# unclearness/vacancy

Measured on AMD Instinct MI355X. Metric: Mvoxel*views/s (Carve), higher is better.
Workload: dtype f32

## Files before the change

### vacancy_amd/csrc/carve_fused.h

```cpp
#pragma once
#include <algorithm>
#include <cstdint>

#include "carve_common.h"

namespace vcy {

#ifndef VCY_WG_WAVES
#define VCY_WG_WAVES 4
#endif
constexpr int kWgWaves = VCY_WG_WAVES;
constexpr int BX = 8 * kWgWaves, BY = 8, BZ = 8;
constexpr int WX = 8;
constexpr int kMaxFusedViews = 64;
constexpr int kTileRaw = 16;
constexpr int kRawBuffers = 2;
template <int TQ>
constexpr int tile_f4_per_wave() { return TQ == kTileRaw ? kRawBuffers * 64 : TQ; }
constexpr int kTileBig = 512;
constexpr int kBigPixels = 4 * kTileBig;

constexpr int kCoopSdfPitch = 8 * VCY_WG_WAVES + 4;
template <typename CountT>
constexpr int coop_cnt_pitch() { return 8 * VCY_WG_WAVES + 16 / (int)sizeof(CountT); }
// ... 56 lines not shown
  float ub;
  int sure;
};
static_assert(sizeof(TileInfo) == 56, "row_lds_bytes_per_wave");

constexpr int kUpdateWaUnitWeight = 2;

struct FootprintRecord {
  uint32_t w0, w1;
};

__device__ __forceinline__ FootprintRecord pack_footprint(const TileInfo& ti, const ViewParams& v) {
  uint32_t b = __float_as_uint(ti.ub);
  if (!(fabsf(ti.ub) <= 3.402823466e+38f)) b = 0x7f800000u;
  else if (b & 0x80000000u) b &= ~63u;
  else b = (b + 63u) & ~63u;
  FootprintRecord r;
  const int tx1 = ti.tx0 + ti.tw - 1, ty1 = ti.ty0 + ti.th - 1;
  r.w0 = b | (uint32_t)ti.th | (ti.nq && tx1 == v.roi_max_xi ? 16u : 0u) | (ti.nq && ty1 == v.roi_max_yi ? 32u : 0u);
  r.w1 = ti.nq ? ((uint32_t)ti.tx0 | ((uint32_t)ti.ty0 << 13) | ((uint32_t)ti.tw << 26) | ((uint32_t)ti.sure << 30)) : 0u;
  return r;
}

__device__ __forceinline__ TileInfo unpack_footprint(const FootprintRecord r) {
  TileInfo ti;
  const int tw = (int)((r.w1 >> 26) & 15u), th = (int)(r.w0 & 15u);
  const int tx0 = (int)(r.w1 & 8191u), ty0 = (int)((r.w1 >> 13) & 8191u);
  ti.ub = __uint_as_float(r.w0 & ~63u);
  ti.sure = (int)(r.w1 >> 30);
  ti.tx0 = tx0, ti.ty0 = ty0, ti.tw = tw, ti.th = (tw ? th : 0), ti.nq = tw * th;
  ti.pitchf = tw ? 16.0f : 0.0f;
  ti.inv_tw = tw ? 0.0625f : 1.0f;
  ti.base = tw ? -(ty0 * 16 + tx0) : 0;
  if (tw) {
    const int tx1 = tx0 + tw - 1, ty1 = ty0 + th - 1;
    ti.lo_x = (float)tx0, ti.lo_y = (float)ty0;
    ti.hi_x = (r.w0 & 16u) ? (float)tx1 : __uint_as_float(__float_as_uint((float)(tx1 + 1)) - 1u);
    ti.hi_y = (r.w0 & 32u) ? (float)ty1 : __uint_as_float(__float_as_uint((float)(ty1 + 1)) - 1u);
  } else {
    ti.lo_x = ti.lo_y = INFINITY;
    ti.hi_x = ti.hi_y = -INFINITY;
    ti.ub = INFINITY;
    ti.sure = 0;
  }
  return ti;
}

struct FastDivU32 {
  uint32_t d, m, s1, s2;
};
__device__ __forceinline__ uint32_t fast_div_u32(uint32_t n, const FastDivU32& f) {
  const uint32_t t = __umulhi(n, f.m);
  return (t + ((n - t) >> f.s1)) >> f.s2;
}
inline FastDivU32 make_fast_div_u32(uint32_t d) {
  FastDivU32 f;
  uint32_t l = 0;
  while ((1ull << l) < d) ++l;
  f.d = d;
  f.m = (uint32_t)((((1ull << l) - d) << 32) / d + 1);
  f.s1 = l < 1 ? l : 1;
  f.s2 = l < 1 ? 0 : l - 1;
  return f;
}

struct BlockDecode {
  int total;
  int layer, q, rem, dealt;
// ... 63 lines not shown
```

### vacancy_amd/csrc/carve_fused_device.h

```cpp
#pragma once
#include "carve_fused.h"

namespace vcy {
namespace {

#define VCY_SETPRIO(n) __builtin_amdgcn_s_setprio(n)

#ifdef VCY_PHASE_TIMING
__device__ unsigned long long g_phase_ticks[256][16];
#define VCY_PT_DECL unsigned long long pt_last = __builtin_amdgcn_s_memtime(), pt_acc[16] = {0, 0, 0, 0, 0, 0, 0, 0, 0, 0, 0, 0, 0, 0, 0, 0}
#define VCY_PT(slot)                                                  \
  do {                                                                \
    const unsigned long long t_ = __builtin_amdgcn_s_memtime();       \
    pt_acc[slot] += t_ - pt_last;                                     \
    pt_last = t_;                                                     \
  } while (0)
#define VCY_PT_COUNT(slot) pt_acc[slot] += 1
#define VCY_PT_FLUSH(lane_)                                                                         \
  do {                                                                                              \
    if ((lane_) == 0)                                                                               \
      for (int q_ = 0; q_ < 16; ++q_) atomicAdd(&g_phase_ticks[blockIdx.x & 255][q_], pt_acc[q_]);  \
  } while (0)
#else
#define VCY_PT_DECL
// ... 120 lines not shown
typedef float f4 __attribute__((ext_vector_type(4)));
typedef f4 __attribute__((address_space(3))) lds_float4;

template <int UPDATE>
__device__ __forceinline__ bool apply_sample(bool ok, float dist, float wgt, float& s, float& fn) {
  const float f1 = fn + 1.0f;
  float avg;
  if (UPDATE == kUpdateWaUnitWeight) {
    avg = (fn * s + dist) * rcp_count(f1);
  } else {
    avg = (wgt * fn * s + wgt * dist) * div_fast(1.0f, wgt * f1);
  }
  const float ns = (fn < 1.0f) ? dist : avg;
  s = ok ? ns : s;
  fn = ok ? f1 : fn;
  return ok;
}

__device__ __forceinline__ int div_small(int q, float inv) { return (int)(((float)q + 0.5f) * inv); }

typedef float __attribute__((address_space(3))) lds_float;
typedef uint32_t __attribute__((address_space(3))) lds_u32;

__device__ __forceinline__ void raw_prefetch(const ViewParams& v, const TileInfo& ti, int lane, float* buf) {
#ifdef VCY_FLOOR_NO_TILE_LOADS
  return;
#endif
  asm volatile("" : "+v"(lane));
  const int nq = __builtin_amdgcn_readfirstlane(ti.nq);
  if (nq == 0) return;
  const int th = __builtin_amdgcn_readfirstlane(ti.th);
  const int tx0 = __builtin_amdgcn_readfirstlane(ti.tx0);
  const int ty0 = __builtin_amdgcn_readfirstlane(ti.ty0);
  gfloat_ptr img = (gfloat_ptr)v.sdf;
  const unsigned width = (unsigned)v.width;
  lds_float* dst = (lds_float*)buf;
  if (tx0 + 15 <= v.roi_max_xi && ty0 + 15 <= v.roi_max_yi) {
    const unsigned lane_off = __umul24(width, (unsigned)lane >> 4) + ((unsigned)lane & 15u);
    gfloat_ptr base = img + (__umul24(width, (unsigned)ty0) + (unsigned)tx0);
#pragma unroll
    for (int r = 0; r < 4; ++r) {
      if (4 * r <= th)
        __builtin_amdgcn_global_load_lds(base + (size_t)(4 * r) * width + lane_off, dst + 64 * r, 4, 0, 0);
    }
    return;
  }
  const unsigned xx = (unsigned)min(tx0 + (lane & 15), v.roi_max_xi);
  const int yl = ty0 + (lane >> 4);
#pragma unroll
  for (int r = 0; r < 4; ++r) {
    if (4 * r <= th) {
      const unsigned yy = (unsigned)min(yl + 4 * r, v.roi_max_yi);
      __builtin_amdgcn_global_load_lds(img + (__umul24(width, yy) + xx), dst + 64 * r, 4, 0, 0);
    }
  }
}

__device__ __forceinline__ void raw_tile_wait() { asm volatile("s_waitcnt vmcnt(0)" ::: "memory"); }

__device__ __forceinline__ float wave_min(float v) {
#define VCY_DPP_MIN(CTRL) "s_nop 1\n\tv_min_f32_dpp %0, %0, %0 " CTRL "\n\t"
  asm volatile(VCY_DPP_MIN("quad_perm:[1,0,3,2] row_mask:0xf bank_mask:0xf")
               VCY_DPP_MIN("quad_perm:[2,3,0,1] row_mask:0xf bank_mask:0xf")
               VCY_DPP_MIN("row_half_mirror row_mask:0xf bank_mask:0xf")
               VCY_DPP_MIN("row_mirror row_mask:0xf bank_mask:0xf")
               VCY_DPP_MIN("row_bcast:15 row_mask:0xa bank_mask:0xf")
               VCY_DPP_MIN("row_bcast:31 row_mask:0xc bank_mask:0xf")
               : "+v"(v));
#undef VCY_DPP_MIN
  return __uint_as_float(__builtin_amdgcn_readlane(__float_as_uint(v), 63));
}

__device__ __forceinline__ void tile_fill(const ViewParams& v, const TileInfo& ti, int lane, float* tile) {
  const int nq = __builtin_amdgcn_readfirstlane(ti.nq);
  if (nq == 0) return;
  const int tw = __builtin_amdgcn_readfirstlane(ti.tw), th = __builtin_amdgcn_readfirstlane(ti.th);
  const int tx0 = __builtin_amdgcn_readfirstlane(ti.tx0);
// ... 208 lines not shown
  uint32_t w32[sizeof(TileInfo) / 4];
  __builtin_memcpy(w32, &ti, sizeof(TileInfo));
  lds_u32* dst = tinfo_lds + vi * (int)(sizeof(TileInfo) / 4);
#pragma unroll
  for (int q = 0; q < (int)(sizeof(TileInfo) / 4); ++q) dst[q] = w32[q];
}

template <bool SAMEF, int TQ, bool GEN>
__device__ __attribute__((noinline)) float brick_footprints(const FusedView* __restrict__ views, int nviews, int lane,
                                                            float xl, float xh, float yl, float yh, float zl_, float zh,
                                                            bool is_ortho, bool outside_max, bool want_bound,
                                                            bool want_lower, lds_u32* tinfo_lds) {
  float ub_lane = INFINITY;
  if (lane < nviews) {
    const FusedView fv = load_fused_view(views, lane);
    const TileInfo ti = footprint_of<SAMEF, TQ, GEN>(fv, xl, xh, yl, yh, zl_, zh, is_ortho, outside_max, want_bound,
                                                     want_lower);
    store_tile_info(tinfo_lds, lane, ti);
    ub_lane = ti.ub;
  }
  return ub_lane;
}

}
}
```

### vacancy_amd/csrc/carve_fused_kernel.h

```cpp
#pragma once
#include <cstdio>
#include <cstdlib>
#include <type_traits>

#include "carve_fused_device.h"

namespace vcy {
namespace {

template <int UPDATE, bool CHECKMAX, int TQ, bool GEN, int NB>
constexpr int carve_waves_per_simd() {
  if (NB > 1) return NB > 2 ? 4 : 5;
  if (GEN || CHECKMAX || TQ != kTileRaw || UPDATE == VCY_UPDATE_WEIGHTED_AVERAGE) return VCY_WAVES_CHECKED;
  if (UPDATE == kUpdateWaUnitWeight) return NB == 0 ? VCY_WAVES_WA_ONE : VCY_WAVES_WA;
  return NB == 0 ? VCY_WAVES_ONE : VCY_WAVES;
}
template <typename CountT, int UPDATE, bool TRUNC, bool SAMEF, bool CHECKMAX, int TQ, bool GEN, int DIV, int NB = 1>
__global__ __launch_bounds__(64 * (NB > 1 ? kRowWaves : kWgWaves))
__attribute__((amdgpu_waves_per_eu(NB > 1 ? 1 : carve_waves_per_simd<UPDATE, CHECKMAX, TQ, GEN, NB>(),
                                   carve_waves_per_simd<UPDATE, CHECKMAX, TQ, GEN, NB>()))) void carve_fused_kernel(GridParams g,
                                                          const FusedView* __restrict__ views,
                                                          const float* __restrict__ c0_all,
                                                          int nviews_arg, ModeParams mode, int nbx,
                                                          int nby, BlockDecode bd, int cull_enabled, int state_flags,
                                                          const FootprintRecord* __restrict__ records,
                                                          int64_t nbricks, float* __restrict__ brick_min,
                                                          const int* __restrict__ wg_list,
                                                          unsigned long long* __restrict__ pair_count) {
  constexpr bool kOne = NB == 0;
  constexpr bool kOneRegs = kOne;
  const int nviews = kOne ? 1 : nviews_arg;
  const int fresh = state_flags & kStateFresh;
  const bool implied = (state_flags & kStateCountImplied) != 0;
  const bool coop = NB <= 1 && (kWgWaves == 4 || kWgWaves == 8) && (state_flags & kStateCoopStore) != 0;
  const bool nt_store = (state_flags & kStateStreamStore) != 0;
  constexpr bool kRows = NB > 1;
  static_assert(!kRows || (TQ == kTileRaw && !CHECKMAX), "the few-view flavour: raw tiles, no update limit in reach");
  extern __shared__ float4 fused_lds[];
  constexpr bool kRaw = TQ == kTileRaw;
  constexpr int kTileF4 = NB == 0 ? 64 : tile_f4_per_wave<TQ>();
  constexpr bool kNeedBound = TRUNC || UPDATE == VCY_UPDATE_MAX;

  VCY_SETPRIO(3);
  const int tid = threadIdx.x;
  const int wave = __builtin_amdgcn_readfirstlane(tid >> 6), lane = tid & 63;
  VCY_PT_DECL;
  constexpr size_t kRowWaveBytes = kRows ? row_lds_bytes_per_wave<CountT, NB>() : 0;
  static_assert(kRowWaveBytes % 16 == 0, "wave regions are 16-byte aligned");
  float4* tile = kRows ? (float4*)((char*)fused_lds + wave * kRowWaveBytes) : fused_lds + wave * kTileF4;
  TileInfo* tinfo = kRows ? (TileInfo*)((char*)tile + kRawBuffers * 1024)
                          : (TileInfo*)(fused_lds + kWgWaves * kTileF4) + wave * nviews;
  float* stage_s = (float*)((char*)tinfo + NB * kRowMaxViews * sizeof(TileInfo));
  CountT* stage_n = (CountT*)(stage_s + NB * 64 * WX);
  typedef unsigned long long __attribute__((address_space(3))) lds_u64_row;
  lds_u64_row* stage_mask = (lds_u64_row*)(unsigned long long*)(stage_n + NB * 64 * WX);
  static_assert((sizeof(TileInfo) * kWgWaves) % 16 == 0, "alignment of the cooperative write-back's staging");
  typedef CountT CountVec8 __attribute__((ext_vector_type(WX)));
  typedef CountVec8 __attribute__((address_space(3))) lds_countvec;
  typedef unsigned long long __attribute__((address_space(3))) lds_u64;
  float* coop_s = NB == 0 ? (float*)(fused_lds + kWgWaves * kTileF4)
                          : (float*)((TileInfo*)(fused_lds + kWgWaves * kTileF4) + kWgWaves * nviews);
  CountT* coop_n = (CountT*)(coop_s + 64 * kCoopSdfPitch);
  lds_u64* coop_mask = (lds_u64*)(unsigned long long*)(coop_n + 64 * coop_cnt_pitch<CountT>());
  auto coop_leave = [&]() {
    if (coop) {
      if (lane == 0) coop_mask[wave] = 0ull, coop_mask[kWgWaves + wave] = 0ull;
      __builtin_amdgcn_fence(__ATOMIC_RELEASE, "workgroup");
    }
  };
  TileInfo ti_one;
  auto tile_of = [&](int p) -> const TileInfo& {
    if constexpr (kOneRegs) return ti_one;
    else return tinfo[p];
  };
  int cur = 0;
  auto raw_buf = [&](int b) -> float* { return (float*)tile + 256 * b; };
  const int ly = lane & (BY - 1), lz = lane >> 3;
  int b = kRows ? ((int)(blockIdx.x & 7u) + 8 * (kRowWaves * (int)(blockIdx.x >> 3) + wave)) : (int)blockIdx.x;
  const int* list_entry = nullptr;
  int list_live = 0;
  FootprintRecord list_rec;
  list_rec.w0 = 0u, list_rec.w1 = 0u;
  if (wg_list != nullptr) {
    if (kRows) b = (int)blockIdx.x * kRowWaves + wave;
    if (b >= wg_list[0]) return;
    if (kOne && (state_flags & kStateListRecords) != 0) {
      list_entry = wg_list + 2 + (int64_t)b * kLiveEntryWords;
      typedef uint32_t u32x2 __attribute__((ext_vector_type(2)));
      typedef const u32x2 __attribute__((address_space(1))) * gent_ptr;
      const u32x2 head = ((gent_ptr)list_entry)[0], mine = ((gent_ptr)list_entry)[1 + wave];
      b = __builtin_amdgcn_readfirstlane((int)head.x);
      list_live = __builtin_amdgcn_readfirstlane((int)head.y);
      list_rec.w0 = (uint32_t)__builtin_amdgcn_readfirstlane((int)mine.x);
      list_rec.w1 = (uint32_t)__builtin_amdgcn_readfirstlane((int)mine.y);
    } else {
      b = wg_list[1 + b];
    }
  } else {
    if (kRows && b >= bd.total) return;
// ... 69 lines not shown
      rec.w0 = raw.x, rec.w1 = raw.y;
      const TileInfo ti = unpack_footprint(rec);
      store_tile_info((lds_u32*)tinfo, lane, ti);
      ub_lane = ti.ub;
    }
  } else if constexpr (kOneRegs) {
    typedef uint32_t u32x2 __attribute__((ext_vector_type(2)));
    typedef const u32x2 __attribute__((address_space(1))) * grec_ptr;
    FootprintRecord rec;
    if (list_entry != nullptr) {
      rec = list_rec;
    } else {
      const u32x2 raw = ((grec_ptr)records)[brick_lin];
      rec.w0 = (uint32_t)__builtin_amdgcn_readfirstlane((int)raw.x), rec.w1 = (uint32_t)__builtin_amdgcn_readfirstlane((int)raw.y);
    }
    ti_one = unpack_footprint(rec);
    ub_lane = ti_one.ub;
  } else if (kRaw && records != nullptr) {
    ub_lane = INFINITY;
    if (lane < nviews) {
      typedef uint32_t u32x2 __attribute__((ext_vector_type(2)));
      typedef const u32x2 __attribute__((address_space(1))) * grec_ptr;
      const u32x2 raw = ((grec_ptr)records)[(int64_t)lane * nbricks + brick_lin];
      FootprintRecord rec;
      rec.w0 = raw.x, rec.w1 = raw.y;
      const TileInfo ti = unpack_footprint(rec);
      store_tile_info((lds_u32*)tinfo, lane, ti);
      ub_lane = ti.ub;
    }
  } else {
    const int x_lo = min(x_first, g.nx - 1), x_hi = min(x_first + WX - 1, g.nx - 1);
    const int y_hi = min(by * BY + BY - 1, g.ny - 1);
    const int z_hi = min(zl0 + BZ - 1, g.nz_local - 1);
    ub_lane = brick_footprints<SAMEF, TQ, GEN>(views, nviews, lane, g.px[x_lo], g.px[x_hi], g.py[by * BY], g.py[y_hi],
                                               g.pz[g.z0 + zl0], g.pz[g.z0 + z_hi], mode.ortho != 0,
                                               mode.outside == VCY_OUTSIDE_MAX, want_bound,
                                               want_bound && TRUNC && UPDATE != VCY_UPDATE_MAX, (lds_u32*)tinfo);
  }
  wave_lds_fence();
#if defined(VCY_DEV_EXIT_AT) && VCY_DEV_EXIT_AT == 2
  {
    coop_leave();
    return;
  }
#endif
  const unsigned long long view_mask = kRows ? __ballot(pair_valid) : ((nviews >= 64) ? ~0ull : ((1ull << nviews) - 1ull));
  unsigned long long live = view_mask;
  if (want_bound && !fresh && !(kOne && list_entry != nullptr)) {
    const bool have_min = UPDATE == VCY_UPDATE_MAX && (state_flags & kStateBrickMinValid) != 0 && brick_min != nullptr;
    if (TRUNC || have_min) {
      bool drop0 = TRUNC && ub_lane < -1.0f;
      if (have_min) {
        float smin0;
        if constexpr (kRows) smin0 = pair_valid ? brick_min[brick_seg + pair_j] : 0.0f;
        else smin0 = ((cfloat_ptr)brick_min)[brick_lin];
        drop0 = drop0 || ub_lane <= smin0;
      }
      live = __ballot(!drop0) & view_mask;
      if (live == 0ull) {
        coop_leave();
        return;
      }
    }
  }
#ifdef VCY_PHASE_TIMING
  {
    asm volatile("" ::"v"(ub_lane));
    const unsigned long long t_ = __builtin_amdgcn_s_memtime();
    pt_acc[13] += t_ - pt_last;
  }
#endif

#if defined(VCY_DEV_EXIT_AT) && VCY_DEV_EXIT_AT == 3
  {
    coop_leave();
    return;
  }
#endif
  CountT* __restrict__ cnt = (CountT*)g.cnt;
  constexpr bool kFloatCount = UPDATE != VCY_UPDATE_MAX;
  typedef typename std::conditional<kFloatCount, float, int>::type NT;
  float s[WX];
  NT n[WX];
  const int64_t row0 = ((int64_t)zl * g.ny + y) * g.nx;
  int vi_pre = -1;
  auto prefetch_first_tile = [&]() {
    if constexpr (kRaw) {
      const bool listed_live = kOne && list_entry != nullptr;
      const bool have_min = UPDATE == VCY_UPDATE_MAX && !fresh && (state_flags & kStateBrickMinValid) != 0 && brick_min != nullptr;
      if (!(fresh || UPDATE != VCY_UPDATE_MAX || !want_bound || have_min || listed_live)) return;
      bool drop = false;
      if (want_bound && !listed_live) {
        if (TRUNC) drop = ub_lane < -1.0f;
        if (have_min) {
          const float smin0 = ((cfloat_ptr)brick_min)[brick_lin];
          if (smin0 != kInvalidSdf) drop = drop || ub_lane <= smin0;
        }
      }
      const unsigned long long lp = __ballot(!drop) & view_mask;
      vi_pre = lp ? (__ffsll((long long)lp) - 1) : nviews;
      if (vi_pre < nviews) raw_prefetch(views[vi_pre].v, tile_of(vi_pre), lane, raw_buf(0));
    }
  };
  const bool vec_io = (g.nx & (WX - 1)) == 0;
  typedef CountT CountVec __attribute__((ext_vector_type(WX)));
  if constexpr (kRows) {
#pragma unroll
    for (int k = 0; k < WX; ++k) {
      s[k] = kInvalidSdf;
      n[k] = (NT)0;
    }
    if (lane < NB) stage_mask[lane] = 0ull;
    if (!fresh) {
      const int yl = min(by * BY + (lane >> 3), g.ny - 1);
      const unsigned off_s = (unsigned)yl * (unsigned)g.nx + (unsigned)(lane & 7);
      constexpr int kCntPerDword = 4 / (int)sizeof(CountT);
      constexpr int kCntDwordsPerRow = WX / kCntPerDword;
      constexpr int kCntRowsPerReq = 64 / kCntDwordsPerRow;
      constexpr int kCntReqs = 64 / kCntRowsPerReq;
      const int crow = lane / kCntDwordsPerRow;
      typedef const CountT __attribute__((address_space(1))) * gcnt_ptr;
#pragma unroll
      for (int j = 0; j < NB; ++j) {
        if (((live >> (8 * j)) & 0xffull) == 0ull) continue;
        const int xb = x_seg + j * WX;
#pragma unroll
        for (int r = 0; r < BZ; ++r) {
          const int zr = min(zl0 + r, g.nz_local - 1);
          gfloat_ptr src = (gfloat_ptr)g.sdf + ((int64_t)zr * g.ny * g.nx + xb);
          __builtin_amdgcn_global_load_lds(src + off_s, (lds_float*)(stage_s + (j * 64 + 8 * r) * WX), 4, 0, 0);
        }
#pragma unroll
        for (int r = 0; r < kCntReqs; ++r) {
          const int row = r * kCntRowsPerReq + crow;
          const int yr = min(by * BY + (row & 7), g.ny - 1), zr = min(zl0 + (row >> 3), g.nz_local - 1);
          gcnt_ptr src = (gcnt_ptr)cnt + (((int64_t)zr * g.ny + yr) * g.nx + xb + (lane % kCntDwordsPerRow) * kCntPerDword);
          __builtin_amdgcn_global_load_lds((const uint32_t __attribute__((address_space(1)))*)src,
                                           (lds_u32*)(uint32_t*)(stage_n + (j * 64 + r * kCntRowsPerReq) * WX), 4, 0, 0);
        }
      }
    }
  } else if (fresh) {
#pragma unroll
    for (int k = 0; k < WX; ++k) {
      s[k] = kInvalidSdf;
      n[k] = (NT)0;
    }
  } else if (vec_io) {
    float4 a, b4;
    CountVec cv;
    if (kOne && eager) {
      a = make_float4(eager_a.x, eager_a.y, eager_a.z, eager_a.w), b4 = make_float4(eager_b.x, eager_b.y, eager_b.z, eager_b.w);
      cv = eager_c;
    } else {
      a = *(const float4*)(g.sdf + row0 + x_first), b4 = *(const float4*)(g.sdf + row0 + x_first + 4);
      cv = *(const CountVec*)(cnt + row0 + x_first);
    }
    prefetch_first_tile();
    s[0] = a.x, s[1] = a.y, s[2] = a.z, s[3] = a.w, s[4] = b4.x, s[5] = b4.y, s[6] = b4.z, s[7] = b4.w;
#pragma unroll
    for (int k = 0; k < WX; ++k) n[k] = (NT)cv[k];
  } else {
#pragma unroll
    for (int k = 0; k < WX; ++k) {
      const int xk = min(x_first + k, g.nx - 1);
      s[k] = g.sdf[row0 + xk];
      n[k] = (NT)cnt[row0 + xk];
    }
  }
// ... 22 lines not shown
    if (fresh) {
      uniform_cnt = true;
      fnu = 0.0f;
    } else {
      const float f0 = __uint_as_float(__builtin_amdgcn_readfirstlane(__float_as_uint((float)n[0])));
      bool same = true;
#pragma unroll
      for (int k = 0; k < WX; ++k) same = same && (float)n[k] == f0;
      uniform_cnt = __all(same);
      fnu = f0;
    }
  };
  if (!kRows) refresh_uniform_cnt();
  auto leave_uniform = [&]() {
    if (!uniform_cnt) return;
    uniform_cnt = false;
#pragma unroll
    for (int k = 0; k < WX; ++k) n[k] = (NT)fnu;
  };
  int jc = -1;
  auto live_views = [&]() -> unsigned long long {
    bool drop = false;
    if (want_bound) {
      if (TRUNC) drop = ub_lane < -1.0f;
      if (UPDATE == VCY_UPDATE_MAX && all_touched) {
        float m = s[0];
#pragma unroll
        for (int k = 1; k < WX; ++k) m = fminf(m, s[k]);
        const float smin = wave_min(m);
        drop = drop || ub_lane <= smin;
      }
    }
    if constexpr (kRows) {
      const unsigned long long cur_bits = 0xffull << (8 * jc);
      return (live & ~cur_bits) | (__ballot(!drop) & view_mask & cur_bits);
    }
    return __ballot(!drop) & view_mask;
  };
  const int vi_end = kRows ? 64 : nviews;
  auto next_view = [&](unsigned long long live, int after) -> int {
    const unsigned long long rest = (after >= 63) ? 0ull : (live & ~((2ull << after) - 1ull));
    return rest ? (__ffsll((long long)rest) - 1) : vi_end;
  };

  unsigned long long changed_lanes = 0ull;
  if (!kRows) live = live_views();
  int vi = live ? (__ffsll((long long)live) - 1) : vi_end;
  if (kRaw && vi < vi_end && vi != vi_pre) raw_prefetch(views[kRows ? (vi & 7) : vi].v, tile_of(vi), lane, raw_buf(0));
  typedef CountT CountVecR __attribute__((ext_vector_type(WX)));
  typedef CountVecR __attribute__((address_space(3))) lds_countvec_r;
  auto finish_brick = [&]() {
    if constexpr (kRows) {
      leave_uniform();
      if (brick_min != nullptr && implied) {
        float m = s[0];
#pragma unroll
        for (int k = 1; k < WX; ++k) m = fminf(m, s[k]);
        const float smin = wave_min(m);
        if (lane == 0) brick_min[brick_lin] = smin;
      }
      lds_float4* rs = (lds_float4*)(float4*)(stage_s + (jc * 64 + lane) * WX);
      rs[0] = f4{s[0], s[1], s[2], s[3]};
      rs[1] = f4{s[4], s[5], s[6], s[7]};
      CountVecR cv;
#pragma unroll
      for (int k = 0; k < WX; ++k) cv[k] = (CountT)n[k];
      *(lds_countvec_r*)(CountVecR*)(stage_n + (jc * 64 + lane) * WX) = cv;
      if (lane == 0) stage_mask[jc] = fresh ? ~0ull : changed_lanes;
    }
  };
  auto begin_brick = [&](int j) {
// ... 38 lines not shown
  const bool is_ortho = GEN && mode.ortho != 0, is_nn = GEN && mode.interp == VCY_INTERP_NN;
  typedef const ViewParams __attribute__((address_space(4))) cview;
  cview* vp = nullptr;
  cfloat_ptr c0 = nullptr;
  int vnext = vi_end;
  float pitchf = 0.0f;
  int base = 0, big_pitch = 0;
  const lds_float* rawcur = nullptr;
  float h12x = 0.0f, h12y = 0.0f, h12z = 0.0f;
  auto begin_view = [&]() {
    const int vv = kRows ? (vi & 7) : vi;
    const ViewParams& v = views[vv].v;
    vp = (cview*)&v;
    c0 = (cfloat_ptr)(c0_all + ((size_t)vv * (nxp / WX) + (x_first / WX)) * kC0Stride);
    VCY_SETPRIO(3);
    wave_lds_fence();
    if (kRaw) {
      raw_tile_wait();
    } else {
      tile_fill(v, tile_of(vi), lane, (float*)tile);
    }
    wave_lds_fence();
    vnext = next_view(live, vi);
    if (kRaw && vnext < vi_end) raw_prefetch(views[kRows ? (vnext & 7) : vnext].v, tile_of(vnext), lane, raw_buf(cur ^ 1));
    ++n_processed;
    pitchf = tile_of(vi).pitchf;
    base = tile_of(vi).base;
    big_pitch = kRaw ? 16 : (int)pitchf;
    rawcur = (const lds_float*)raw_buf(cur);
    h12x = vp->r[0][1] * py + vp->r[0][2] * pz, h12y = vp->r[1][1] * py + vp->r[1][2] * pz;
    h12z = vp->r[2][1] * py + vp->r[2][2] * pz;
    VCY_SETPRIO(0);
    VCY_PT(1);
  };
  auto end_view = [&](bool brick_moved) {
    VCY_SETPRIO(3);
    if (brick_moved) VCY_PT_COUNT(11);
    none_touched = false;
    if (!kOne) refresh_all_touched();

    if (!kOne && want_bound && UPDATE == VCY_UPDATE_MAX && brick_moved) {
      live = live_views();
      const int v2 = next_view(live, vi);
      if (v2 != vnext) {
        vnext = v2;
        if (kRaw && vnext < vi_end) raw_prefetch(views[kRows ? (vnext & 7) : vnext].v, tile_of(vnext), lane, raw_buf(cur ^ 1));
      }
    }
    vi = vnext;
    cur ^= 1;
    VCY_PT(5);
  };
  auto next_fast_bits = [&]() -> int {
    if (kOne || vi >= vi_end) return 0;
    if (kRows && (vi >> 3) != jc) return 0;
    const int bits = __builtin_amdgcn_readfirstlane(tile_of(vi).sure);
    return (bits & 1) != 0 ? bits : 0;
  };
  while (vi < vi_end) {
    if constexpr (kRows) {
      if ((vi >> 3) != jc) {
        raw_tile_wait();
        wave_lds_fence();
        if (jc >= 0) finish_brick();
        begin_brick(vi >> 3);
        live = live_views();
        if (((live >> vi) & 1ull) == 0ull) {
          vi = next_view(live, vi);
          if (vi < vi_end) raw_prefetch(views[vi & 7].v, tile_of(vi), lane, raw_buf(cur));
          continue;
        }
      }
    }
    begin_view();
    auto quad_at = [&](unsigned idx) -> float4 {
      if constexpr (kRaw) {
        const lds_float* p = rawcur + idx;
        return make_float4(p[0], p[1], p[16], p[17]);
      } else {
        const lds_float* p = (const lds_float*)(float*)tile + idx;
        const lds_float* p2 = p + big_pitch;
        return make_float4(p[0], p[1], p2[0], p2[1]);
      }
    };

    auto carve_view = [&](auto sure_tag) {
      constexpr bool SURE = decltype(sure_tag)::value;
      cview& v = *vp;
      const float lo_x = tile_of(vi).lo_x, hi_x = tile_of(vi).hi_x;
      const float lo_y = tile_of(vi).lo_y, hi_y = tile_of(vi).hi_y;
      bool slow[WX];
      bool any_slow = false;
      bool moved = false;
#pragma unroll
      for (int k = 0; k < WX; ++k) {
        const float pcz = v.t[2] + (c0[16 + k] + h12z);
        float qx = 1.0f, qy = 1.0f;
        if (!is_ortho) {
          qx = div_view<DIV>(v.fx, pcz);
          qy = SAMEF ? qx : div_view<DIV>(v.fy, pcz);
        }
        const float pcx = v.t[0] + (c0[2 * k] + h12x), pcy = v.t[1] + (c0[2 * k + 1] + h12y);
        const float u = is_ortho ? pcx : qx * pcx + v.cx;
        const float w = is_ortho ? pcy : qy * pcy + v.cy;
        bool in_tile = true;
        if (!SURE) {
          const bool zfast = is_ortho ? !(pcz < 0.0f) : in_fast_div_range(pcz);
          in_tile = zfast && u >= lo_x && u <= hi_x && w >= lo_y && w <= hi_y;
          slow[k] = !in_tile;
          any_slow = any_slow || !in_tile;
        }
        const float fu = floorf(u), fw = floorf(w);
        const float lu = u - fu, lv = w - fw;
// ... 98 lines not shown
            if (is_nn) {
              const float top = lu[j] >= 0.5f ? q[j].y : q[j].x, bot = lu[j] >= 0.5f ? q[j].w : q[j].z;
              dist = lv[j] >= 0.5f ? bot : top;
            }
          }
          if constexpr (FIRST) {
            s[k] = dist;
            n[k] = (NT)1;
          } else if constexpr (kFastMax) {
            update_max_touched(dist, s[k], n[k], took);
          } else if constexpr (UNIFORM) {
            if constexpr (UPDATE == kUpdateWaUnitWeight) s[k] = (fn_v * s[k] + dist) * inv_v;
            else s[k] = (fn_v * s[k] + wgt_v * dist) * inv_v;
          } else if constexpr (kFastWa) {
            update_wa_unit<TRUNC && !NOTRUNC>(dist, s[k], n[k], took);
          }
        }
      }
      constexpr bool kConditional = !FIRST && !UNIFORM && (kFastMax || (kFastWa && TRUNC && !NOTRUNC));
      changed_lanes |= kConditional ? took : ~0ull;
      return (kFastMax && !FIRST) ? took != 0ull : true;
    };
    bool brick_moved;
    const int sure_bits = __builtin_amdgcn_readfirstlane(tile_of(vi).sure);
    const bool sure = (sure_bits & 1) != 0, never_truncated = (sure_bits & 2) != 0;
    const bool fast_first = kFastMax && sure && none_touched;
    const bool fast_next = (kFastMax && sure && all_touched) || (kFastWa && sure && implied);
    const bool fast_general = kFastWaGeneral && sure && uniform_cnt && (!TRUNC || never_truncated);
    if (kFastWaGeneral && __builtin_expect_with_probability(fast_general, 1, 0.9)) {
      if (fnu < 1.0f) {
        brick_moved = carve_view_fast(std::true_type{}, std::false_type{}, std::false_type{});
        fnu = 1.0f;
      } else {
        brick_moved = carve_view_fast(std::false_type{}, std::true_type{}, std::true_type{});
      }
      VCY_PT(2);
      VCY_PT_COUNT(7);
    } else if (kFastMax && __builtin_expect_with_probability(fast_next || fast_first, 1, 0.99)) {
      auto run = [&](auto first_tag) -> bool {
        brick_moved = carve_view_fast(first_tag, std::false_type{}, std::false_type{});
        VCY_PT(2);
        VCY_PT_COUNT(7);
        end_view(brick_moved);
        if (!all_touched || (next_fast_bits() & 1) == 0) return false;
        begin_view();
        return true;
      };
      bool more = true;
      if (fast_first) more = run(std::true_type{});
      while (more) more = run(std::false_type{});
      continue;
// ... 34 lines not shown
#pragma unroll
      for (int i = 0; i < BZ; ++i) {
        const int row = 8 * i + (lane >> 3);
        if (zl0 + i < g.nz_local && col_ok && ((mw >> row) & 1ull) != 0ull) {
          const f4 q = *(const lds_float4*)(float4*)(stage_s + (jw * 64 + row) * WX + (c16 & 1) * 4);
          *(float4*)(g.sdf + (((int64_t)(zl0 + i) * g.ny + yw) * g.nx + x_seg + 4 * c16)) = make_float4(q.x, q.y, q.z, q.w);
        }
      }
      const int jn = lane & 3;
      const unsigned long long mn = jn < NB ? stage_mask[jn] : 0ull;
#pragma unroll
      for (int i = 0; i < 4; ++i) {
        const int row = 16 * i + (lane >> 2);
        const int yn = by * BY + (row & 7), zn = zl0 + (row >> 3);
        if (jn < NB && yn < g.ny && zn < g.nz_local && x_seg + WX * jn < g.nx && ((mn >> row) & 1ull) != 0ull) {
          const CountVecR cv = *(const lds_countvec_r*)(CountVecR*)(stage_n + (jn * 64 + row) * WX);
          *(CountVecR*)(cnt + (((int64_t)zn * g.ny + yn) * g.nx + x_seg + WX * jn)) = cv;
        }
      }
    }
    return;
  }
  leave_uniform();
  int tid_w = (int)threadIdx.x;
  asm volatile("" : "+v"(tid_w));
  const int lane_w = tid_w & 63;
  const int y_w = by * BY + (lane_w & (BY - 1)), zl_w = zl0 + (lane_w >> 3);
  const bool lane_valid_w = y_w < g.ny && zl_w < g.nz_local;
  const int64_t row0_w = ((int64_t)min(zl_w, g.nz_local - 1) * g.ny + min(y_w, g.ny - 1)) * g.nx;
#if defined(VCY_DEV_EXIT_AT) && VCY_DEV_EXIT_AT == 5
  {
    coop_leave();
    return;
  }
#endif
  if (pair_count != nullptr && lane == 0) atomicAdd(&pair_count[bz], (unsigned long long)n_processed);
  if (brick_min != nullptr && implied) {
    float m = s[0];
#pragma unroll
    for (int k = 1; k < WX; ++k) m = fminf(m, s[k]);
    const float smin = wave_min(m);
    if (lane == 0) brick_min[brick_lin] = smin;
  }
  if (coop) {
    const bool changed = lane_valid_w && (fresh != 0 || ((changed_lanes >> lane_w) & 1ull) != 0ull);
    const unsigned long long my_mask = __ballot(changed);
// ... 58 lines not shown
        *(CountVec*)(cnt + row0_w + x_first) = cv;
      }
    } else {
#pragma unroll
      for (int k = 0; k < WX; ++k) {
        if (x_first + k < g.nx) {
          const int64_t idx = row0_w + x_first + k;
          if (fresh || ((changed_lanes >> lane_w) & 1ull) != 0ull) {
            g.sdf[idx] = s[k];
            cnt[idx] = (CountT)n[k];
          }
        }
      }
    }
  }
  VCY_PT(6);
  VCY_PT_FLUSH(lane);
}

template <typename CountT, int UPDATE, bool TRUNC, bool SAMEF, bool CHECKMAX, int TQ, bool GEN, int DIV, int NB>
void launch_instance(const CarveLaunch& l) {
  constexpr bool kRows = NB > 1;
  const size_t coop = (l.state_flags & kStateCoopStore) ? coop_lds_bytes<CountT>() : 0;
  const size_t lds = kRows    ? (size_t)kRowWaves * row_lds_bytes_per_wave<CountT, NB>()
                     : NB == 0 ? (size_t)kWgWaves * 64 * sizeof(float4) + coop
                               : (size_t)kWgWaves * tile_f4_per_wave<TQ>() * sizeof(float4) +
                                     (size_t)kWgWaves * l.n_views * sizeof(TileInfo) + coop;
  const BlockDecode bd = make_block_decode(kRows ? (unsigned)l.row_units : l.grid_x, l.nbx, l.nby);
  hipLaunchKernelGGL((carve_fused_kernel<CountT, UPDATE, TRUNC, SAMEF, CHECKMAX, TQ, GEN, DIV, NB>), dim3(l.grid_x),
                     dim3(64 * (kRows ? kRowWaves : kWgWaves)), lds, l.stream, l.g, l.views, l.c0_all,
                     NB == 0 ? 1 : l.n_views, l.mode, l.nbx, l.nby, bd, l.cull, l.state_flags, l.records, l.nbricks,
                     l.brick_min, l.wg_list, l.pair_count);
}

template <int... Vs, typename F>
void with_constant(int value, F&& f) {
  if (!((value == Vs && (f(std::integral_constant<int, Vs>{}), true)) || ...)) {
    fprintf(stderr, "carve_fused_kernel: no instance for selection %d\n", value);
    abort();
  }
}

template <typename CountT>
void launch_fused(const CarveLaunch& l) {
  const int nb = l.flavour == CarveFlavour::kGeneral ? 1 : (l.flavour == CarveFlavour::kOneView ? 0 : kRowBricks);
#ifdef VCY_DEV_BENCH_KERNELS_ONLY
  if (l.big || l.checkmax || l.gen || l.div_level != 2 || !l.samef || sizeof(CountT) != 1 ||
      l.update == VCY_UPDATE_WEIGHTED_AVERAGE) {
    fprintf(stderr, "VCY_DEV_BENCH_KERNELS_ONLY: kernel variant not built\n");
    abort();
// ... 37 lines not shown
```

Measured before the change: 4.513 million.

## Keep packed per-view footprint records in VGPRs instead of LDS TileInfo

For the max-update raw-tile general flavour, each lane now holds its view's packed 8-byte footprint record in registers and other lanes read it via readlane. Tile bounds, base and sure bits are unpacked on demand. This removes the per-view TileInfo array from LDS and its store and fence traffic, which shrinks LDS use per workgroup. It also defers filling fresh voxel state until it is actually needed. In exchange there is extra scalar unpack arithmetic in the per-view loop, and a noinline helper is added that computes records in place.

```diff
diff --git a/vacancy_amd/csrc/carve_fused.h b/vacancy_amd/csrc/carve_fused.h
--- a/vacancy_amd/csrc/carve_fused.h
+++ b/vacancy_amd/csrc/carve_fused.h
@@ -102,11 +102,14 @@
   return r;
 }
 
-__device__ __forceinline__ TileInfo unpack_footprint(const FootprintRecord r) {
+__host__ __device__ __forceinline__ float bits_as_float(uint32_t b) { return __builtin_bit_cast(float, b); }
+__host__ __device__ __forceinline__ uint32_t float_as_bits(float f) { return __builtin_bit_cast(uint32_t, f); }
+
+__host__ __device__ __forceinline__ TileInfo unpack_footprint(const FootprintRecord r) {
   TileInfo ti;
   const int tw = (int)((r.w1 >> 26) & 15u), th = (int)(r.w0 & 15u);
   const int tx0 = (int)(r.w1 & 8191u), ty0 = (int)((r.w1 >> 13) & 8191u);
-  ti.ub = __uint_as_float(r.w0 & ~63u);
+  ti.ub = bits_as_float(r.w0 & ~63u);
   ti.sure = (int)(r.w1 >> 30);
   ti.tx0 = tx0, ti.ty0 = ty0, ti.tw = tw, ti.th = (tw ? th : 0), ti.nq = tw * th;
   ti.pitchf = tw ? 16.0f : 0.0f;
@@ -115,8 +118,8 @@
   if (tw) {
     const int tx1 = tx0 + tw - 1, ty1 = ty0 + th - 1;
     ti.lo_x = (float)tx0, ti.lo_y = (float)ty0;
-    ti.hi_x = (r.w0 & 16u) ? (float)tx1 : __uint_as_float(__float_as_uint((float)(tx1 + 1)) - 1u);
-    ti.hi_y = (r.w0 & 32u) ? (float)ty1 : __uint_as_float(__float_as_uint((float)(ty1 + 1)) - 1u);
+    ti.hi_x = (r.w0 & 16u) ? (float)tx1 : bits_as_float(float_as_bits((float)(tx1 + 1)) - 1u);
+    ti.hi_y = (r.w0 & 32u) ? (float)ty1 : bits_as_float(float_as_bits((float)(ty1 + 1)) - 1u);
   } else {
     ti.lo_x = ti.lo_y = INFINITY;
     ti.hi_x = ti.hi_y = -INFINITY;
@@ -124,6 +127,43 @@
     ti.sure = 0;
   }
   return ti;
+}
+
+struct FootprintFields {
+  int tx0, ty0, tw, th, nq;
+  int sure;
+  int edge;
+};
+struct FootprintBounds {
+  float lo_x, hi_x, lo_y, hi_y;
+};
+__host__ __device__ __forceinline__ uint32_t footprint_ub_word(uint32_t w0, uint32_t w1) {
+  return ((w1 >> 26) & 15u) ? w0 : 0x7f800000u;
+}
+__host__ __device__ __forceinline__ float footprint_ub(uint32_t ub_word) { return bits_as_float(ub_word & ~63u); }
+__host__ __device__ __forceinline__ FootprintFields unpack_footprint_scalar(uint32_t ub_word, uint32_t w1) {
+  FootprintFields f;
+  const int th = (int)(ub_word & 15u);
+  f.tw = (int)((w1 >> 26) & 15u);
+  f.tx0 = (int)(w1 & 8191u), f.ty0 = (int)((w1 >> 13) & 8191u);
+  f.th = f.tw ? th : 0, f.nq = f.tw * th;
+  f.sure = f.tw ? (int)(w1 >> 30) : 0;
+  f.edge = (int)((ub_word >> 4) & 3u);
+  return f;
+}
+__host__ __device__ __forceinline__ int footprint_base(const FootprintFields& f) { return f.tw ? -(f.ty0 * 16 + f.tx0) : 0; }
+__host__ __device__ __forceinline__ FootprintBounds footprint_bounds(const FootprintFields& f) {
+  FootprintBounds b;
+  if (f.tw) {
+    const int tx1 = f.tx0 + f.tw - 1, ty1 = f.ty0 + f.th - 1;
+    b.lo_x = (float)f.tx0, b.lo_y = (float)f.ty0;
+    b.hi_x = (f.edge & 1) ? (float)tx1 : bits_as_float(float_as_bits((float)(tx1 + 1)) - 1u);
+    b.hi_y = (f.edge & 2) ? (float)ty1 : bits_as_float(float_as_bits((float)(ty1 + 1)) - 1u);
+  } else {
+    b.lo_x = b.lo_y = INFINITY;
+    b.hi_x = b.hi_y = -INFINITY;
+  }
+  return b;
 }
 
 struct FastDivU32 {
diff --git a/vacancy_amd/csrc/carve_fused_device.h b/vacancy_amd/csrc/carve_fused_device.h
--- a/vacancy_amd/csrc/carve_fused_device.h
+++ b/vacancy_amd/csrc/carve_fused_device.h
@@ -166,6 +166,30 @@
 typedef float __attribute__((address_space(3))) lds_float;
 typedef uint32_t __attribute__((address_space(3))) lds_u32;
 
+__device__ __forceinline__ void raw_prefetch_rows(const ViewParams& v, int th, int tx0, int ty0, int lane, float* buf) {
+  gfloat_ptr img = (gfloat_ptr)v.sdf;
+  const unsigned width = (unsigned)v.width;
+  lds_float* dst = (lds_float*)buf;
+  if (tx0 + 15 <= v.roi_max_xi && ty0 + 15 <= v.roi_max_yi) {
+    const unsigned lane_off = __umul24(width, (unsigned)lane >> 4) + ((unsigned)lane & 15u);
+    gfloat_ptr base = img + (__umul24(width, (unsigned)ty0) + (unsigned)tx0);
+#pragma unroll
+    for (int r = 0; r < 4; ++r) {
+      if (4 * r <= th)
+        __builtin_amdgcn_global_load_lds(base + (size_t)(4 * r) * width + lane_off, dst + 64 * r, 4, 0, 0);
+    }
+    return;
+  }
+  const unsigned xx = (unsigned)min(tx0 + (lane & 15), v.roi_max_xi);
+  const int yl = ty0 + (lane >> 4);
+#pragma unroll
+  for (int r = 0; r < 4; ++r) {
+    if (4 * r <= th) {
+      const unsigned yy = (unsigned)min(yl + 4 * r, v.roi_max_yi);
+      __builtin_amdgcn_global_load_lds(img + (__umul24(width, yy) + xx), dst + 64 * r, 4, 0, 0);
+    }
+  }
+}
 __device__ __forceinline__ void raw_prefetch(const ViewParams& v, const TileInfo& ti, int lane, float* buf) {
 #ifdef VCY_FLOOR_NO_TILE_LOADS
   return;
@@ -176,27 +200,40 @@
   const int th = __builtin_amdgcn_readfirstlane(ti.th);
   const int tx0 = __builtin_amdgcn_readfirstlane(ti.tx0);
   const int ty0 = __builtin_amdgcn_readfirstlane(ti.ty0);
+  raw_prefetch_rows(v, th, tx0, ty0, lane, buf);
+}
+__device__ __forceinline__ void raw_prefetch(const ViewParams& v, const FootprintFields& f, int lane, float* buf) {
+#ifdef VCY_FLOOR_NO_TILE_LOADS
+  return;
+#endif
+  asm volatile("" : "+v"(lane));
+  if (f.nq == 0) return;
   gfloat_ptr img = (gfloat_ptr)v.sdf;
   const unsigned width = (unsigned)v.width;
   lds_float* dst = (lds_float*)buf;
-  if (tx0 + 15 <= v.roi_max_xi && ty0 + 15 <= v.roi_max_yi) {
+  const int groups = (f.th >> 2) + 1;
+  if (f.tx0 + 15 <= v.roi_max_xi && f.ty0 + 15 <= v.roi_max_yi) {
     const unsigned lane_off = __umul24(width, (unsigned)lane >> 4) + ((unsigned)lane & 15u);
-    gfloat_ptr base = img + (__umul24(width, (unsigned)ty0) + (unsigned)tx0);
-#pragma unroll
-    for (int r = 0; r < 4; ++r) {
-      if (4 * r <= th)
-        __builtin_amdgcn_global_load_lds(base + (size_t)(4 * r) * width + lane_off, dst + 64 * r, 4, 0, 0);
+    gfloat_ptr base = img + (__umul24(width, (unsigned)f.ty0) + (unsigned)f.tx0);
+    switch (groups) {
+      default: __builtin_amdgcn_global_load_lds(base + (size_t)12 * width + lane_off, dst + 192, 4, 0, 0); [[fallthrough]];
+      case 3: __builtin_amdgcn_global_load_lds(base + (size_t)8 * width + lane_off, dst + 128, 4, 0, 0); [[fallthrough]];
+      case 2: __builtin_amdgcn_global_load_lds(base + (size_t)4 * width + lane_off, dst + 64, 4, 0, 0); [[fallthrough]];
+      case 1: __builtin_amdgcn_global_load_lds(base + lane_off, dst, 4, 0, 0);
     }
     return;
   }
-  const unsigned xx = (unsigned)min(tx0 + (lane & 15), v.roi_max_xi);
-  const int yl = ty0 + (lane >> 4);
-#pragma unroll
-  for (int r = 0; r < 4; ++r) {
-    if (4 * r <= th) {
-      const unsigned yy = (unsigned)min(yl + 4 * r, v.roi_max_yi);
-      __builtin_amdgcn_global_load_lds(img + (__umul24(width, yy) + xx), dst + 64 * r, 4, 0, 0);
-    }
+  const unsigned xx = (unsigned)min(f.tx0 + (lane & 15), v.roi_max_xi);
+  const int yl = f.ty0 + (lane >> 4);
+  auto row = [&](int r) {
+    const unsigned yy = (unsigned)min(yl + 4 * r, v.roi_max_yi);
+    __builtin_amdgcn_global_load_lds(img + (__umul24(width, yy) + xx), dst + 64 * r, 4, 0, 0);
+  };
+  switch (groups) {
+    default: row(3); [[fallthrough]];
+    case 3: row(2); [[fallthrough]];
+    case 2: row(1); [[fallthrough]];
+    case 1: row(0);
   }
 }
 
@@ -451,5 +488,22 @@
   return ub_lane;
 }
 
-}
-}
+template <bool SAMEF, bool GEN>
+__device__ __attribute__((noinline)) FootprintRecord brick_footprint_records(const FusedView* __restrict__ views, int nviews,
+                                                                             int lane, float xl, float xh, float yl, float yh,
+                                                                             float zl_, float zh, bool is_ortho,
+                                                                             bool outside_max, bool want_bound,
+                                                                             bool want_lower) {
+  FootprintRecord rec;
+  rec.w0 = 0x7f800000u, rec.w1 = 0u;
+  if (lane < nviews) {
+    const FusedView fv = load_fused_view(views, lane);
+    const TileInfo ti = footprint_of<SAMEF, kTileRaw, GEN>(fv, xl, xh, yl, yh, zl_, zh, is_ortho, outside_max, want_bound,
+                                                            want_lower);
+    rec = pack_footprint(ti, fv.v);
+  }
+  return rec;
+}
+
+}
+}
diff --git a/vacancy_amd/csrc/carve_fused_kernel.h b/vacancy_amd/csrc/carve_fused_kernel.h
--- a/vacancy_amd/csrc/carve_fused_kernel.h
+++ b/vacancy_amd/csrc/carve_fused_kernel.h
@@ -14,6 +14,10 @@
   if (GEN || CHECKMAX || TQ != kTileRaw || UPDATE == VCY_UPDATE_WEIGHTED_AVERAGE) return VCY_WAVES_CHECKED;
   if (UPDATE == kUpdateWaUnitWeight) return NB == 0 ? VCY_WAVES_WA_ONE : VCY_WAVES_WA;
   return NB == 0 ? VCY_WAVES_ONE : VCY_WAVES;
+}
+template <int UPDATE, int TQ, int NB>
+constexpr bool carve_keeps_records() {
+  return UPDATE == VCY_UPDATE_MAX && TQ == kTileRaw && NB == 1;
 }
 template <typename CountT, int UPDATE, bool TRUNC, bool SAMEF, bool CHECKMAX, int TQ, bool GEN, int DIV, int NB = 1>
 __global__ __launch_bounds__(64 * (NB > 1 ? kRowWaves : kWgWaves))
@@ -38,6 +42,7 @@
   static_assert(!kRows || (TQ == kTileRaw && !CHECKMAX), "the few-view flavour: raw tiles, no update limit in reach");
   extern __shared__ float4 fused_lds[];
   constexpr bool kRaw = TQ == kTileRaw;
+  constexpr bool kRecRegs = carve_keeps_records<UPDATE, TQ, NB>();
   constexpr int kTileF4 = NB == 0 ? 64 : tile_f4_per_wave<TQ>();
   constexpr bool kNeedBound = TRUNC || UPDATE == VCY_UPDATE_MAX;
 
@@ -58,8 +63,8 @@
   typedef CountT CountVec8 __attribute__((ext_vector_type(WX)));
   typedef CountVec8 __attribute__((address_space(3))) lds_countvec;
   typedef unsigned long long __attribute__((address_space(3))) lds_u64;
-  float* coop_s = NB == 0 ? (float*)(fused_lds + kWgWaves * kTileF4)
-                          : (float*)((TileInfo*)(fused_lds + kWgWaves * kTileF4) + kWgWaves * nviews);
+  float* coop_s = (NB == 0 || kRecRegs) ? (float*)(fused_lds + kWgWaves * kTileF4)
+                                        : (float*)((TileInfo*)(fused_lds + kWgWaves * kTileF4) + kWgWaves * nviews);
   CountT* coop_n = (CountT*)(coop_s + 64 * kCoopSdfPitch);
   lds_u64* coop_mask = (lds_u64*)(unsigned long long*)(coop_n + 64 * coop_cnt_pitch<CountT>());
   auto coop_leave = [&]() {
@@ -73,8 +78,22 @@
     if constexpr (kOneRegs) return ti_one;
     else return tinfo[p];
   };
+  uint32_t rec_w0 = 0x7f800000u, rec_w1 = 0u;
+  auto rec_of = [&](int p) -> FootprintFields {
+    return unpack_footprint_scalar((uint32_t)__builtin_amdgcn_readlane((int)rec_w0, p),
+                                   (uint32_t)__builtin_amdgcn_readlane((int)rec_w1, p));
+  };
   int cur = 0;
   auto raw_buf = [&](int b) -> float* { return (float*)tile + 256 * b; };
+  auto prefetch_tile = [&](int p, float* buf) {
+    const ViewParams& v = views[kRows ? (p & 7) : p].v;
+    if constexpr (kRecRegs) raw_prefetch(v, rec_of(p), lane, buf);
+    else raw_prefetch(v, tile_of(p), lane, buf);
+  };
+  auto sure_of = [&](int p) -> int {
+    if constexpr (kRecRegs) return rec_of(p).sure;
+    else return __builtin_amdgcn_readfirstlane(tile_of(p).sure);
+  };
   const int ly = lane & (BY - 1), lz = lane >> 3;
   int b = kRows ? ((int)(blockIdx.x & 7u) + 8 * (kRowWaves * (int)(blockIdx.x >> 3) + wave)) : (int)blockIdx.x;
   const int* list_entry = nullptr;
@@ -190,12 +209,25 @@
       typedef uint32_t u32x2 __attribute__((ext_vector_type(2)));
       typedef const u32x2 __attribute__((address_space(1))) * grec_ptr;
       const u32x2 raw = ((grec_ptr)records)[(int64_t)lane * nbricks + brick_lin];
-      FootprintRecord rec;
-      rec.w0 = raw.x, rec.w1 = raw.y;
-      const TileInfo ti = unpack_footprint(rec);
-      store_tile_info((lds_u32*)tinfo, lane, ti);
-      ub_lane = ti.ub;
-    }
+      if constexpr (kRecRegs) {
+        rec_w0 = footprint_ub_word(raw.x, raw.y), rec_w1 = raw.y;
+      } else {
+        FootprintRecord rec;
+        rec.w0 = raw.x, rec.w1 = raw.y;
+        const TileInfo ti = unpack_footprint(rec);
+        store_tile_info((lds_u32*)tinfo, lane, ti);
+        ub_lane = ti.ub;
+      }
+    }
+  } else if constexpr (kRecRegs) {
+    const int x_lo = min(x_first, g.nx - 1), x_hi = min(x_first + WX - 1, g.nx - 1);
+    const int y_hi = min(by * BY + BY - 1, g.ny - 1);
+    const int z_hi = min(zl0 + BZ - 1, g.nz_local - 1);
+    const FootprintRecord rec = brick_footprint_records<SAMEF, GEN>(
+        views, nviews, lane, g.px[x_lo], g.px[x_hi], g.py[by * BY], g.py[y_hi], g.pz[g.z0 + zl0], g.pz[g.z0 + z_hi],
+        mode.ortho != 0, mode.outside == VCY_OUTSIDE_MAX, want_bound, want_bound && TRUNC && UPDATE != VCY_UPDATE_MAX);
+    rec_w0 = footprint_ub_word(rec.w0, rec.w1), rec_w1 = rec.w1;
+    ub_lane = INFINITY;
   } else {
     const int x_lo = min(x_first, g.nx - 1), x_hi = min(x_first + WX - 1, g.nx - 1);
     const int y_hi = min(by * BY + BY - 1, g.ny - 1);
@@ -205,6 +237,10 @@
                                                mode.outside == VCY_OUTSIDE_MAX, want_bound,
                                                want_bound && TRUNC && UPDATE != VCY_UPDATE_MAX, (lds_u32*)tinfo);
   }
+  auto lane_ub = [&]() -> float {
+    if constexpr (kRecRegs) return footprint_ub(rec_w0);
+    else return ub_lane;
+  };
   wave_lds_fence();
 #if defined(VCY_DEV_EXIT_AT) && VCY_DEV_EXIT_AT == 2
   {
@@ -217,12 +253,12 @@
   if (want_bound && !fresh && !(kOne && list_entry != nullptr)) {
     const bool have_min = UPDATE == VCY_UPDATE_MAX && (state_flags & kStateBrickMinValid) != 0 && brick_min != nullptr;
     if (TRUNC || have_min) {
-      bool drop0 = TRUNC && ub_lane < -1.0f;
+      bool drop0 = TRUNC && lane_ub() < -1.0f;
       if (have_min) {
         float smin0;
         if constexpr (kRows) smin0 = pair_valid ? brick_min[brick_seg + pair_j] : 0.0f;
         else smin0 = ((cfloat_ptr)brick_min)[brick_lin];
-        drop0 = drop0 || ub_lane <= smin0;
+        drop0 = drop0 || lane_ub() <= smin0;
       }
       live = __ballot(!drop0) & view_mask;
       if (live == 0ull) {
@@ -233,7 +269,7 @@
   }
 #ifdef VCY_PHASE_TIMING
   {
-    asm volatile("" ::"v"(ub_lane));
+    asm volatile("" ::"v"(lane_ub()));
     const unsigned long long t_ = __builtin_amdgcn_s_memtime();
     pt_acc[13] += t_ - pt_last;
   }
@@ -250,6 +286,20 @@
   typedef typename std::conditional<kFloatCount, float, int>::type NT;
   float s[WX];
   NT n[WX];
+  constexpr bool kLazyFresh = UPDATE == VCY_UPDATE_MAX && !TRUNC && !CHECKMAX && NB == 1;
+  bool state_set = true;
+  auto set_fresh_state = [&]() {
+    if constexpr (kLazyFresh) {
+      if (!state_set) {
+#pragma unroll
+        for (int k = 0; k < WX; ++k) {
+          s[k] = kInvalidSdf;
+          n[k] = (NT)0;
+        }
+        state_set = true;
+      }
+    }
+  };
   const int64_t row0 = ((int64_t)zl * g.ny + y) * g.nx;
   int vi_pre = -1;
   auto prefetch_first_tile = [&]() {
@@ -259,15 +309,15 @@
       if (!(fresh || UPDATE != VCY_UPDATE_MAX || !want_bound || have_min || listed_live)) return;
       bool drop = false;
       if (want_bound && !listed_live) {
-        if (TRUNC) drop = ub_lane < -1.0f;
+        if (TRUNC) drop = lane_ub() < -1.0f;
         if (have_min) {
           const float smin0 = ((cfloat_ptr)brick_min)[brick_lin];
-          if (smin0 != kInvalidSdf) drop = drop || ub_lane <= smin0;
+          if (smin0 != kInvalidSdf) drop = drop || lane_ub() <= smin0;
         }
       }
       const unsigned long long lp = __ballot(!drop) & view_mask;
       vi_pre = lp ? (__ffsll((long long)lp) - 1) : nviews;
-      if (vi_pre < nviews) raw_prefetch(views[vi_pre].v, tile_of(vi_pre), lane, raw_buf(0));
+      if (vi_pre < nviews) prefetch_tile(vi_pre, raw_buf(0));
     }
   };
   const bool vec_io = (g.nx & (WX - 1)) == 0;
@@ -309,10 +359,14 @@
       }
     }
   } else if (fresh) {
-#pragma unroll
-    for (int k = 0; k < WX; ++k) {
-      s[k] = kInvalidSdf;
-      n[k] = (NT)0;
+    if constexpr (kLazyFresh) {
+      state_set = false;
+    } else {
+#pragma unroll
+      for (int k = 0; k < WX; ++k) {
+        s[k] = kInvalidSdf;
+        n[k] = (NT)0;
+      }
     }
   } else if (vec_io) {
     float4 a, b4;
@@ -381,13 +435,13 @@
   auto live_views = [&]() -> unsigned long long {
     bool drop = false;
     if (want_bound) {
-      if (TRUNC) drop = ub_lane < -1.0f;
+      if (TRUNC) drop = lane_ub() < -1.0f;
       if (UPDATE == VCY_UPDATE_MAX && all_touched) {
         float m = s[0];
 #pragma unroll
         for (int k = 1; k < WX; ++k) m = fminf(m, s[k]);
         const float smin = wave_min(m);
-        drop = drop || ub_lane <= smin;
+        drop = drop || lane_ub() <= smin;
       }
     }
     if constexpr (kRows) {
@@ -405,7 +459,7 @@
   unsigned long long changed_lanes = 0ull;
   if (!kRows) live = live_views();
   int vi = live ? (__ffsll((long long)live) - 1) : vi_end;
-  if (kRaw && vi < vi_end && vi != vi_pre) raw_prefetch(views[kRows ? (vi & 7) : vi].v, tile_of(vi), lane, raw_buf(0));
+  if (kRaw && vi < vi_end && vi != vi_pre) prefetch_tile(vi, raw_buf(0));
   typedef CountT CountVecR __attribute__((ext_vector_type(WX)));
   typedef CountVecR __attribute__((address_space(3))) lds_countvec_r;
   auto finish_brick = [&]() {
@@ -490,10 +544,13 @@
     }
     wave_lds_fence();
     vnext = next_view(live, vi);
-    if (kRaw && vnext < vi_end) raw_prefetch(views[kRows ? (vnext & 7) : vnext].v, tile_of(vnext), lane, raw_buf(cur ^ 1));
+    if (kRaw && vnext < vi_end) prefetch_tile(vnext, raw_buf(cur ^ 1));
     ++n_processed;
-    pitchf = tile_of(vi).pitchf;
-    base = tile_of(vi).base;
+    if constexpr (kRecRegs) {
+      pitchf = (float)kTileRaw, base = footprint_base(rec_of(vi));
+    } else {
+      pitchf = tile_of(vi).pitchf, base = tile_of(vi).base;
+    }
     big_pitch = kRaw ? 16 : (int)pitchf;
     rawcur = (const lds_float*)raw_buf(cur);
     h12x = vp->r[0][1] * py + vp->r[0][2] * pz, h12y = vp->r[1][1] * py + vp->r[1][2] * pz;
@@ -512,7 +569,7 @@
       const int v2 = next_view(live, vi);
       if (v2 != vnext) {
         vnext = v2;
-        if (kRaw && vnext < vi_end) raw_prefetch(views[kRows ? (vnext & 7) : vnext].v, tile_of(vnext), lane, raw_buf(cur ^ 1));
+        if (kRaw && vnext < vi_end) prefetch_tile(vnext, raw_buf(cur ^ 1));
       }
     }
     vi = vnext;
@@ -522,7 +579,7 @@
   auto next_fast_bits = [&]() -> int {
     if (kOne || vi >= vi_end) return 0;
     if (kRows && (vi >> 3) != jc) return 0;
-    const int bits = __builtin_amdgcn_readfirstlane(tile_of(vi).sure);
+    const int bits = sure_of(vi);
     return (bits & 1) != 0 ? bits : 0;
   };
   while (vi < vi_end) {
@@ -535,7 +592,7 @@
         live = live_views();
         if (((live >> vi) & 1ull) == 0ull) {
           vi = next_view(live, vi);
-          if (vi < vi_end) raw_prefetch(views[vi & 7].v, tile_of(vi), lane, raw_buf(cur));
+          if (vi < vi_end) prefetch_tile(vi, raw_buf(cur));
           continue;
         }
       }
@@ -555,8 +612,14 @@
     auto carve_view = [&](auto sure_tag) {
       constexpr bool SURE = decltype(sure_tag)::value;
       cview& v = *vp;
-      const float lo_x = tile_of(vi).lo_x, hi_x = tile_of(vi).hi_x;
-      const float lo_y = tile_of(vi).lo_y, hi_y = tile_of(vi).hi_y;
+      float lo_x, hi_x, lo_y, hi_y;
+      if constexpr (kRecRegs) {
+        const FootprintBounds fb = footprint_bounds(rec_of(vi));
+        lo_x = fb.lo_x, hi_x = fb.hi_x, lo_y = fb.lo_y, hi_y = fb.hi_y;
+      } else {
+        lo_x = tile_of(vi).lo_x, hi_x = tile_of(vi).hi_x;
+        lo_y = tile_of(vi).lo_y, hi_y = tile_of(vi).hi_y;
+      }
       bool slow[WX];
       bool any_slow = false;
       bool moved = false;
@@ -701,11 +764,13 @@
       return (kFastMax && !FIRST) ? took != 0ull : true;
     };
     bool brick_moved;
-    const int sure_bits = __builtin_amdgcn_readfirstlane(tile_of(vi).sure);
+    const int sure_bits = sure_of(vi);
     const bool sure = (sure_bits & 1) != 0, never_truncated = (sure_bits & 2) != 0;
     const bool fast_first = kFastMax && sure && none_touched;
     const bool fast_next = (kFastMax && sure && all_touched) || (kFastWa && sure && implied);
     const bool fast_general = kFastWaGeneral && sure && uniform_cnt && (!TRUNC || never_truncated);
+    if (kLazyFresh && fast_first) state_set = true;
+    else set_fresh_state();
     if (kFastWaGeneral && __builtin_expect_with_probability(fast_general, 1, 0.9)) {
       if (fnu < 1.0f) {
         brick_moved = carve_view_fast(std::true_type{}, std::false_type{}, std::false_type{});
@@ -786,6 +851,7 @@
     return;
   }
   leave_uniform();
+  set_fresh_state();
   int tid_w = (int)threadIdx.x;
   asm volatile("" : "+v"(tid_w));
   const int lane_w = tid_w & 63;
@@ -890,10 +956,11 @@
 void launch_instance(const CarveLaunch& l) {
   constexpr bool kRows = NB > 1;
   const size_t coop = (l.state_flags & kStateCoopStore) ? coop_lds_bytes<CountT>() : 0;
+  constexpr bool rec_regs = carve_keeps_records<UPDATE, TQ, NB>();
   const size_t lds = kRows    ? (size_t)kRowWaves * row_lds_bytes_per_wave<CountT, NB>()
                      : NB == 0 ? (size_t)kWgWaves * 64 * sizeof(float4) + coop
                                : (size_t)kWgWaves * tile_f4_per_wave<TQ>() * sizeof(float4) +
-                                     (size_t)kWgWaves * l.n_views * sizeof(TileInfo) + coop;
+                                     (rec_regs ? 0 : (size_t)kWgWaves * l.n_views * sizeof(TileInfo)) + coop;
   const BlockDecode bd = make_block_decode(kRows ? (unsigned)l.row_units : l.grid_x, l.nbx, l.nby);
   hipLaunchKernelGGL((carve_fused_kernel<CountT, UPDATE, TRUNC, SAMEF, CHECKMAX, TQ, GEN, DIV, NB>), dim3(l.grid_x),
                      dim3(64 * (kRows ? kRowWaves : kWgWaves)), lds, l.stream, l.g, l.views, l.c0_all,
```

Result: faster. 4.576 million (median of 6 runs) (+1.4%).
